# MIC-DKFZ/MultiTalent

Measured on AMD Instinct MI355X. Metric: CT patches/s (48x192x192) train fwd+bwd, higher is better.
Workload: dtype f32; 1 GPU; Task009_Spleen Generic_UNet nc=2 softmax Dice+CE; batch_per_gpu=2, global_batch=2, parallelism=dp1, step=fwd+loss+bwd+clip12+SGD-nesterov, precision=fp32

## Files before the change

### include/mtseg.h

```cpp
#ifndef MTSEG_H
#define MTSEG_H

#include <stddef.h>
#include <stdint.h>

#ifdef __cplusplus
extern "C" {
#endif

#define MT_OK 0
#define MT_EINVAL (-1)
#define MT_EWORKSPACE (-2)
#define MT_EHIP (-3)
#define MT_EUNSUPPORTED (-4)

#define MT_ABI_VERSION 4
#define MT_MAX_CHUNKS 64

#define MT_F32 0
#define MT_BF16 1
#define MT_F16 2

typedef void* mt_stream_t;

// ... 90 lines not shown
                         long s_ci, long s_co, long s_kd, long s_kh, long s_kw, int accumulate,
                         void* workspace, size_t workspace_bytes, mt_stream_t stream);

typedef struct {
  mt_src_t src;
  int32_t N, Db, Hb, Wb;
  int32_t Di, Hi, Wi;
  int32_t siD, siH, siW;
  int32_t soD, soH, soW;
  int32_t Cin, Cout;
  const float* wpack;
  const float* bias;
  float* out; int32_t ocs;
  int32_t accumulate;
  float* stats_part;
  int32_t odtype;
  int32_t scatter;
  int32_t mma;
} mt_pointwise_t;
int mt_pointwise_fwd(const mt_pointwise_t* p, mt_stream_t stream);
int mt_pointwise_stats_blocks(const mt_pointwise_t* p);
int mt_pointwise_io_supported(const mt_pointwise_t* p);
int mt_pointwise_pack_layout(const mt_pointwise_t* p);
int mt_pointwise_kernel_name(const mt_pointwise_t* p, char* buf, size_t n);
int mt_pointwise_launch_shape(const mt_pointwise_t* p, int32_t shape[4]);
int mt_head_bwd_supported(int Cin, int Cout);
size_t mt_head_bwd_workspace(int N, long V, int Cin, int Cout);
int mt_head_bwd(const mt_src_t* x, const float* dy, int dycs, int N, long V, int Cin, int Cout, const float* wpack_bwd,
                float* dx, int dxcs, int dxdtype , int accumulate_dx, float* dw,
                long s_ci, long s_co, float* dbias, int accumulate_dw, int* dbias_done, void* ws, size_t ws_bytes, mt_stream_t stream);
int mt_head_bwd_io_supported(int xdtype, int xcs, int dxdtype, int dxcs, int Cin, int Cout);
int mt_head_bwd_kernel_name(const mt_src_t* x, int dycs, int N, long V, int Cin, int Cout, int dxcs, int dxdtype, char* buf, size_t n,
                            int* dbias_done);


int mt_inorm_finalize(const float* part, int N, int nsb, int C, double count, const float* gamma,
                      const float* beta, float eps, float* mean, float* rstd, float* scale, float* shift,
                      mt_stream_t stream);
int mt_inorm_lrelu_apply(const float* y, int ycs, const float* scale, const float* shift, float slope,
                         const float* res, int rcs, const float* rscale, const float* rshift, float rslope,
                         float* out, int ocs, int N, long V, int C, int dtype , mt_stream_t stream);
size_t mt_inorm_bwd_workspace(int N, long V, int C);
int mt_inorm_lrelu_bwd(float* g, int gcs, const float* y, int ycs, const float* mean, const float* rstd,
                       const float* gamma, const float* beta, float slope, int N, long V, int C,
                       float* dgamma, float* dbeta, float* dbias, const float* part, int part_nblk, int part_cs, int part_c0,
                       void* ws, size_t ws_bytes, int gdtype, int ydtype , mt_stream_t stream);
int mt_lrelu_bwd(float* g, int gcs, const float* y, int ycs, const float* scale, const float* shift,
                 float slope, const float* y2, int y2cs, const float* scale2, const float* shift2,
                 float slope2, float* gcopy, int gcopycs, int N, long V, int C, int gdtype , int ydtype ,
                 mt_stream_t stream);
int mt_lrelu_bwd_stats_blocks(long V, int C);
int mt_lrelu_bwd_stats(float* g, const float* y, const float* scale, const float* shift, float slope,
                       const float* y2, const float* scale2, const float* shift2, float slope2, float* gcopy,
                       const float* mean, const float* rstd, float* part, int N, long V, int C, int gdtype ,
                       int ydtype , mt_stream_t stream);
int mt_inorm_lrelu_apply_kernel_name(const float* y, int ycs, const float* res, int rcs, const float* out, int ocs, int N, long V, int C,
                                     int dtype, char* buf, size_t n);
int mt_inorm_lrelu_bwd_kernel_name(const float* g, int gcs, const float* y, int ycs, const float* mean, const float* rstd, int N, long V, int C,
                                   const float* part, int part_nblk, int part_cs, int part_c0, int gdtype, int ydtype,
                                   char* buf, size_t n, int* own_reduce, int* block);
int mt_lrelu_bwd_kernel_name(const float* g, int gcs, const float* y, int ycs, const float* y2, int y2cs, const float* gcopy, int gcopycs,
                             int N, long V, int C, int gdtype, int ydtype, char* buf, size_t n);
int mt_lrelu_bwd_stats_kernel_name(const float* g, const float* y, const float* y2, const float* gcopy, const float* mean, const float* rstd,
                                   const float* part, int N, long V, int C, int gdtype, int ydtype, char* buf, size_t n);
size_t mt_channel_sum_workspace(int N, long V, int C);
int mt_channel_sum(const float* x, int xcs, int N, long V, int C, float* out, int accumulate,
// ... 194 lines not shown
```

### multitalent_amd/_lib.py

```python
import ctypes as C
import os

_HERE = os.path.dirname(os.path.abspath(__file__))
LIB_PATH = os.path.join(_HERE, os.environ.get('MT_LIB_VARIANT', 'libmtseg_hip.so'))

MT_MAX_CHUNKS = 64
c_float_p = C.POINTER(C.c_float)


class mt_src_t(C.Structure):
    _fields_ = [('ptr', C.c_void_p), ('cs', C.c_int32), ('C', C.c_int32), ('scale', C.c_void_p),
                ('shift', C.c_void_p), ('slope', C.c_float), ('dtype', C.c_int32)]


class mt_bwd_stats_t(C.Structure):
    _fields_ = [('y', C.c_void_p), ('mean', C.c_void_p), ('rstd', C.c_void_p), ('gamma', C.c_void_p), ('beta', C.c_void_p),
                ('ycs', C.c_int32), ('c0', C.c_int32), ('C', C.c_int32), ('slope', C.c_float)]


class mt_conv3d_t(C.Structure):
    _fields_ = [('src', mt_src_t * 2), ('nsrc', C.c_int32),
                ('N', C.c_int32), ('Di', C.c_int32), ('Hi', C.c_int32), ('Wi', C.c_int32),
                ('dilD', C.c_int32), ('dilH', C.c_int32), ('dilW', C.c_int32),
                ('Do', C.c_int32), ('Ho', C.c_int32), ('Wo', C.c_int32),
# ... 44 lines not shown

_vp, _i, _l, _f, _d, _sz = C.c_void_p, C.c_int, C.c_long, C.c_float, C.c_double, C.c_size_t
_P = C.POINTER

SIGNATURES = {
    'mt_last_error': (C.c_char_p, []),
    'mt_abi_version': (_i, []),
    'mt_probe_device': (_i, [_vp, _sz, _P(_i), C.c_char_p, _sz, _vp]),
    'mt_pack_conv_weights': (_i, [_vp, _vp, _P(_sz), _i, _i, _i, _i, _i, _i, _l, _l, _l, _l, _l, _i, _i, _i, _vp, _vp]),
    'mt_conv3d_fwd': (_i, [_P(mt_conv3d_t), _vp]),
    'mt_conv3d_stats_blocks': (_i, [_P(mt_conv3d_t)]),
    'mt_conv3d_ck': (_i, [_P(mt_conv3d_t)]),
    'mt_pack_desc_size': (_sz, []),
    'mt_pack_desc_fill': (_i, [_vp, _vp, _vp, _i, _i, _i, _i, _i, _i, _l, _l, _l, _l, _l, _i, _i, _i, _vp]),
    'mt_pack_batched': (_i, [_vp, _i, _vp]),
    'mt_conv3d_bwd_data_strided': (_i, [_P(mt_conv3d_t), _vp]),
    'mt_conv3d_bwd_data_strided_supported': (_i, [_P(mt_conv3d_t)]),
    'mt_downsample_seg_nearest': (_i, [_vp, _i, _i, _i, _i, _vp, _i, _i, _i, _i, _vp]),
    'mt_gaussian_blur_axis': (_i, [_vp, _vp, _i, _i, _i, _i, _i, _vp, _vp]),
    'mt_conv3d_pack_layout': (_i, [_P(mt_conv3d_t)]),
    'mt_conv3d_bwd_data_strided_pack_layout': (_i, [_P(mt_conv3d_t)]),
    'mt_conv3d_kernel_name': (_i, [_P(mt_conv3d_t), C.c_char_p, _sz]),
    'mt_conv3d_bwd_stats_supported': (_i, [_P(mt_conv3d_t)]),
    'mt_conv3d_bwd_weight_kernel_name': (_i, [_P(mt_conv3d_t), _P(mt_src_t), C.c_char_p, _sz]),
    'mt_conv3d_bwd_data_strided_kernel_name': (_i, [_P(mt_conv3d_t), C.c_char_p, _sz]),
    'mt_conv3d_bwd_weight_workspace': (_sz, [_P(mt_conv3d_t)]),
    'mt_conv3d_bwd_weight': (_i, [_P(mt_conv3d_t), _P(mt_src_t), _vp, _l, _l, _l, _l, _l, _i, _vp, _sz, _vp]),
    'mt_pointwise_fwd': (_i, [_P(mt_pointwise_t), _vp]),
    'mt_pointwise_stats_blocks': (_i, [_P(mt_pointwise_t)]),
    'mt_head_bwd_supported': (_i, [_i, _i]),
    'mt_head_bwd_workspace': (_sz, [_i, _l, _i, _i]),
    'mt_head_bwd': (_i, [_P(mt_src_t), _vp, _i, _i, _l, _i, _i, _vp, _vp, _i, _i, _i, _vp, _l, _l, _vp, _i, _P(C.c_int), _vp, _sz, _vp]),
    'mt_head_bwd_io_supported': (_i, [_i, _i, _i, _i, _i, _i]),
    'mt_pointwise_io_supported': (_i, [_P(mt_pointwise_t)]),
    'mt_pointwise_pack_layout': (_i, [_P(mt_pointwise_t)]),
    'mt_pointwise_kernel_name': (_i, [_P(mt_pointwise_t), C.c_char_p, _sz]),
    'mt_pointwise_launch_shape': (_i, [_P(mt_pointwise_t), _P(C.c_int32)]),
    'mt_head_bwd_kernel_name': (_i, [_P(mt_src_t), _i, _i, _l, _i, _i, _i, _i, C.c_char_p, _sz, _P(C.c_int)]),
    'mt_inorm_finalize': (_i, [_vp, _i, _i, _i, _d, _vp, _vp, _f, _vp, _vp, _vp, _vp, _vp]),
    'mt_inorm_lrelu_apply': (_i, [_vp, _i, _vp, _vp, _f, _vp, _i, _vp, _vp, _f, _vp, _i, _i, _l, _i, _i, _vp]),
    'mt_inorm_bwd_workspace': (_sz, [_i, _l, _i]),
    'mt_inorm_lrelu_bwd': (_i, [_vp, _i, _vp, _i, _vp, _vp, _vp, _vp, _f, _i, _l, _i, _vp, _vp, _vp, _vp, _i, _i, _i, _vp, _sz, _i, _i, _vp]),
    'mt_lrelu_bwd': (_i, [_vp, _i, _vp, _i, _vp, _vp, _f, _vp, _i, _vp, _vp, _f, _vp, _i, _i, _l, _i, _i, _i, _vp]),
    'mt_lrelu_bwd_stats_blocks': (_i, [_l, _i]),
    'mt_lrelu_bwd_stats': (_i, [_vp, _vp, _vp, _vp, _f, _vp, _vp, _vp, _f, _vp, _vp, _vp, _vp, _i, _l, _i, _i, _i, _vp]),
    'mt_inorm_lrelu_apply_kernel_name': (_i, [_vp, _i, _vp, _i, _vp, _i, _i, _l, _i, _i, C.c_char_p, _sz]),
    'mt_inorm_lrelu_bwd_kernel_name': (_i, [_vp, _i, _vp, _i, _vp, _vp, _i, _l, _i, _vp, _i, _i, _i, _i, _i, C.c_char_p, _sz, _P(C.c_int), _P(C.c_int)]),
    'mt_lrelu_bwd_kernel_name': (_i, [_vp, _i, _vp, _i, _vp, _i, _vp, _i, _i, _l, _i, _i, _i, C.c_char_p, _sz]),
    'mt_lrelu_bwd_stats_kernel_name': (_i, [_vp, _vp, _vp, _vp, _vp, _vp, _vp, _i, _l, _i, _i, _i, C.c_char_p, _sz]),
    'mt_channel_sum_workspace': (_sz, [_i, _l, _i]),
    'mt_channel_sum': (_i, [_vp, _i, _i, _l, _i, _vp, _i, _vp, _sz, _i, _vp]),
    'mt_cast': (_i, [_vp, _i, _i, _vp, _i, _i, _l, _i, _i, _vp]),
    'mt_conv3d_io_supported': (_i, [_P(mt_conv3d_t)]),
    'mt_conv3d_bwd_data_strided_io_supported': (_i, [_P(mt_conv3d_t)]),
    'mt_conv3d_bwd_weight_io_supported': (_i, [_P(mt_conv3d_t), _P(mt_src_t)]),
    'mt_multitalent_loss_fwd': (_i, [_vp, _i, _vp, _i, _l, _i, _vp, _vp, _vp, _vp, _sz, _vp]),
    'mt_loss_workspace': (_sz, [_i, _l, _i]),
    'mt_multitalent_loss_bwd': (_i, [_vp, _i, _vp, _i, _l, _i, _vp, _vp, _vp, _vp, _i, _vp]),
    'mt_multitalent_hard_stats': (_i, [_vp, _i, _vp, _i, _l, _i, _vp, _vp, _vp, _vp, _sz, _vp]),
    'mt_hard_stats_workspace': (_sz, [_i, _i]),
    'mt_softmax_dice_ce_fwd': (_i, [_vp, _i, _vp, _i, _l, _i, _vp, _vp, _sz, _vp]),
    'mt_softmax_dice_ce_bwd': (_i, [_vp, _i, _vp, _i, _l, _i, _vp, _vp, _i, _vp]),
    'mt_loss_combine': (_i, [_vp, _vp, _i, _i, _i, _i, _vp, _vp, _i, _i, _f, _f, _f, _f, _f, _vp, _vp, _vp]),
    'mt_multitalent_loss_fwd_kernel_name': (_i, [_i, _l, _i, C.c_char_p, _sz, _P(C.c_long), _P(C.c_int)]),
    'mt_multitalent_loss_bwd_kernel_name': (_i, [_vp, _i, _vp, _i, _l, _i, C.c_char_p, _sz, _P(C.c_long), _P(C.c_int)]),
    'mt_softmax_dice_ce_kernel_name': (_i, [_i, _i, C.c_char_p, _sz]),
# ... 126 lines not shown
```

### multitalent_amd/csrc/head_bwd.hip

```cpp
#include "pw_common.h"
#include <stdio.h>

struct HeadBwdParams {
  mt_src_t x; const float* dy; int dycs; int N; long V; int Cin, Cout;
  const float* wpack; float* dx; int dxcs; int accumulate_dx;
  float* part; int nwaves; long ntiles;
};
template <int NCI, int XS = MT_F32, int OS = MT_F32, bool ST = false>
__global__ __launch_bounds__(256) void head_bwd_kernel(const HeadBwdParams P) {
  constexpr int XE = mt_ebytes<XS>(), OE = mt_ebytes<OS>();
  constexpr int HB_WF = 2048 + 1024 * NCI;
  __shared__ __attribute__((aligned(16))) float hb_img[ST ? 4 * HB_WF : 4];
  static_assert(!ST || 4 * HB_WF * sizeof(float) <= 65536, "head_bwd_kernel: the four wave images must fit the 64 KiB of static LDS (NCI <= 2)");
  const int tid = threadIdx.x, lane = tid & 63;
  const int wave = __builtin_amdgcn_readfirstlane(tid >> 6);
  float* const idy = hb_img + (ST ? wave * HB_WF : 0);
  float* const ixf = idy + (ST ? 2048 : 0);
  const int li = lane & 31, lhalf = lane >> 5;
  const int gw = blockIdx.x * 4 + wave;
  const mt_src_t& S = P.x;
  const bool aff = S.scale != nullptr;
  const float slope = aff ? S.slope : 1.f;
  const int nchunks = (P.Cout + 15) / 16;
  f32x4 wb[NCI][4][2];
// ... 236 lines not shown
  const int row = (j & 3) + 8 * (j >> 2) + 4 * (lane >> 5), col = lane & 31;
  const int ci = t * 32 + row, co = n * 32 + col;
  const bool is_bias = (R.Cin % 32) != 0 && t == R.nci - 1 && row == 31;
  if (co >= R.Cout || (ci >= R.Cin && !is_bias)) return;
  double a = 0.0;
  for (int sl = 0; sl < HB_SLICES; ++sl) a += R.tmp[(size_t)sl * per + e];
  const float s = (float)a;
  if (is_bias) { if (R.dbias != nullptr) R.dbias[co] = R.accumulate ? R.dbias[co] + s : s; return; }
  float* o = R.dw + (long)ci * R.s_ci + (long)co * R.s_co;
  *o = R.accumulate ? *o + s : s;
}

#define HN_BLOCKS 1024
template <int CIN, int ST>
__device__ __forceinline__ void hn_row_from_lds(const char* row, float (&x)[CIN + 2]) {
  if constexpr (ST == MT_F32) {
#pragma unroll
    for (int q = 0; q < CIN / 2; ++q) { const float2 t = *(const float2*)(row + q * 8); x[2 * q] = t.x; x[2 * q + 1] = t.y; }
  } else {
#pragma unroll
    for (int q = 0; q < CIN / 2; ++q) { const unsigned d = *(const unsigned*)(row + q * 4); x[2 * q] = mt_lo16<ST>(d); x[2 * q + 1] = mt_hi16<ST>(d); }
  }
}
template <int CIN, int ST>
__device__ __forceinline__ void hn_row_to_lds(char* row, const float (&x)[CIN + 2]) {
  if constexpr (ST == MT_F32) {
#pragma unroll
    for (int q = 0; q < CIN / 2; ++q) { float2 t; t.x = x[2 * q]; t.y = x[2 * q + 1]; *(float2*)(row + q * 8) = t; }
  } else {
#pragma unroll
    for (int q = 0; q < CIN / 2; ++q) *(unsigned*)(row + q * 4) = mt_pk16<ST>(x[2 * q], x[2 * q + 1]);
  }
}
template <int CIN, int NCO, int XS = MT_F32, int OS = MT_F32>
__global__ __launch_bounds__(256) void head_bwd_narrow_kernel(const HeadBwdParams P) {
  static_assert(CIN % 2 == 0, "channel pairs");
  __shared__ __attribute__((aligned(16))) float hn_img[4 * 64 * CIN];
  constexpr int XE = mt_ebytes<XS>(), OE = mt_ebytes<OS>();
  constexpr int NP = NCO * CIN + NCO;
  __shared__ __attribute__((aligned(16))) float sw[NCO][CIN + 2], ssc[CIN + 2], ssh[CIN + 2];
  __shared__ float red[4][NP];
  const int tid = threadIdx.x, lane = tid & 63;
  const int wave = __builtin_amdgcn_readfirstlane(tid >> 6);
  const mt_src_t& S = P.x;
  const bool aff = S.scale != nullptr;
  const float slope = aff ? S.slope : 1.f;
  for (int i = tid; i < NCO * CIN; i += 256) {
    const int co = i / CIN, ci = i - co * CIN;
    sw[co][ci] = co < P.Cout ? P.wpack[ci * 4 + co] : 0.f;
  }
  float part[NP];
#pragma unroll
  for (int k = 0; k < NP; ++k) part[k] = 0.f;
  const long per_sample_blocks = HN_BLOCKS / P.N > 0 ? HN_BLOCKS / P.N : 1;
  const int nb = (int)(blockIdx.x / per_sample_blocks);
  if (nb < P.N) {
    const long b = blockIdx.x - (long)nb * per_sample_blocks;
    for (int i = tid; i < CIN; i += 256) {
      ssc[i] = aff ? S.scale[(size_t)nb * S.C + i] : 1.f;
      ssh[i] = aff ? S.shift[(size_t)nb * S.C + i] : 0.f;
    }
    __syncthreads();
    const size_t xs = (size_t)P.V * CIN;
    __amdgpu_buffer_rsrc_t ra = __builtin_amdgcn_make_buffer_rsrc((void*)((const char*)S.ptr + (size_t)nb * xs * XE), 0, (int)(xs * XE), 0x00020000);
    __amdgpu_buffer_rsrc_t rx = __builtin_amdgcn_make_buffer_rsrc((void*)((char*)P.dx + (size_t)nb * xs * OE), 0, (int)(xs * OE), 0x00020000);
    const float* dyp = P.dy + (size_t)nb * P.V * P.dycs;
    constexpr int ROWX = CIN * XE, ROWO = CIN * OE;
    constexpr int NPX = 64 * ROWX / 16, NPO = 64 * ROWO / 16;
    char* const img = (char*)hn_img + wave * (64 * CIN * 4);
    for (long v0 = b * 256 + wave * 64; v0 < P.V; v0 += per_sample_blocks * 256) {
      const long v = v0 + lane;
      const bool vok = v < P.V;
      float x[CIN + 2], old[CIN + 2], dy[NCO];
      {
        uint4 pc[(NPX + 63) / 64];
#pragma unroll
        for (int k = 0; k < (NPX + 63) / 64; ++k) {
          const int p = k * 64 + lane;
          pc[k] = __builtin_bit_cast(uint4, __builtin_amdgcn_raw_buffer_load_b128(ra, p < NPX ? (int)(v0 * ROWX) + p * 16 : (int)0x80000000, 0, 0));
        }
#pragma unroll
        for (int k = 0; k < (NPX + 63) / 64; ++k) {
          const int p = k * 64 + lane;
          if (p < NPX) *(uint4*)(img + p * 16) = pc[k];
        }
        __builtin_amdgcn_s_waitcnt(0xc07f);
        __builtin_amdgcn_wave_barrier();
        hn_row_from_lds<CIN, XS>(img + lane * ROWX, x);
        __builtin_amdgcn_s_waitcnt(0xc07f);
        __builtin_amdgcn_wave_barrier();
      }
      if (P.accumulate_dx) {
        uint4 pc[(NPO + 63) / 64];
#pragma unroll
        for (int k = 0; k < (NPO + 63) / 64; ++k) {
          const int p = k * 64 + lane;
          pc[k] = __builtin_bit_cast(uint4, __builtin_amdgcn_raw_buffer_load_b128(rx, p < NPO ? (int)(v0 * ROWO) + p * 16 : (int)0x80000000, 0, 0));
        }
#pragma unroll
        for (int k = 0; k < (NPO + 63) / 64; ++k) {
          const int p = k * 64 + lane;
          if (p < NPO) *(uint4*)(img + p * 16) = pc[k];
        }
        __builtin_amdgcn_s_waitcnt(0xc07f);
        __builtin_amdgcn_wave_barrier();
        hn_row_from_lds<CIN, OS>(img + lane * ROWO, old);
        __builtin_amdgcn_s_waitcnt(0xc07f);
        __builtin_amdgcn_wave_barrier();
      }
#pragma unroll
      for (int co = 0; co < NCO; ++co) dy[co] = (vok && co < P.Cout) ? dyp[v * P.dycs + co] : 0.f;
      float dx[CIN + 2];
#pragma unroll
      for (int ci = 0; ci < CIN; ++ci) {
        const float t = fmaf(x[ci], ssc[ci], ssh[ci]);
        const float a = fmaxf(t, t * slope);
        float g = P.accumulate_dx ? old[ci] : 0.f;
#pragma unroll
        for (int co = 0; co < NCO; ++co) {
          g = fmaf(dy[co], sw[co][ci], g);
          part[co * CIN + ci] = fmaf(a, dy[co], part[co * CIN + ci]);
        }
        dx[ci] = g;
      }
#pragma unroll
      for (int co = 0; co < NCO; ++co) part[NCO * CIN + co] += dy[co];
      hn_row_to_lds<CIN, OS>(img + lane * ROWO, dx);
      __builtin_amdgcn_s_waitcnt(0xc07f);
      __builtin_amdgcn_wave_barrier();
#pragma unroll
      for (int k = 0; k < (NPO + 63) / 64; ++k) {
        const int p = k * 64 + lane;
        if (p < NPO) {
          const uint4 q = *(const uint4*)(img + p * 16);
          __builtin_amdgcn_raw_buffer_store_b128(__builtin_bit_cast(__attribute__((ext_vector_type(4))) unsigned, q), rx, (int)(v0 * ROWO) + p * 16, 0, 0);
        }
      }
      __builtin_amdgcn_s_waitcnt(0xc07f);
      __builtin_amdgcn_wave_barrier();
    }
  }
#pragma unroll
  for (int k = 0; k < NP; ++k) {
    float s = part[k];
#pragma unroll
    for (int off = 32; off > 0; off >>= 1) s += __shfl_xor(s, off, 64);
    if (lane == 0) red[wave][k] = s;
  }
  __syncthreads();
  for (int k = tid; k < NP; k += 256) P.part[(size_t)blockIdx.x * NP + k] = (red[0][k] + red[1][k]) + (red[2][k] + red[3][k]);
}
__global__ __launch_bounds__(64) void head_narrow_reduce_kernel(const float* part, int nblocks, int np, int Cin, int Cout, int nco, float* dw, long s_ci,
                                                               long s_co, float* dbias, int accumulate) {
  const int k = blockIdx.x;
  double s = 0.0;
  for (int b = threadIdx.x; b < nblocks; b += 64) s += (double)part[(size_t)b * np + k];
  s = mt_wave_sum_d(s);
  if (threadIdx.x != 0) return;
  const int co = k < nco * Cin ? k / Cin : k - nco * Cin, ci = k < nco * Cin ? k - co * Cin : -1;
  if (co >= Cout) return;
  if (ci >= 0) { float* o = dw + (long)ci * s_ci + (long)co * s_co; *o = accumulate ? *o + (float)s : (float)s; }
  else if (dbias != nullptr) dbias[co] = accumulate ? dbias[co] + (float)s : (float)s;
}

extern "C" int mt_head_bwd_supported(int Cin, int Cout) { return Cin >= 1 && Cin <= 32 && Cout >= 1 && Cout <= 64; }
extern "C" int mt_head_bwd_io_supported(int xdtype, int xcs, int dxdtype, int dxcs, int Cin, int Cout) {
  if (xdtype == MT_F32 && dxdtype == MT_F32) return 1;
  if (!(mt_is16(xdtype) && dxdtype == MT_BF16)) return 0;
  return ((Cin & 1) || (xcs & 1) || (dxcs & 1)) ? 0 : 1;
}
static inline int head_bwd_waves(int N, long V) {
  const long ntiles = (long)N * ((V + 31) / 32);
  long w = ntiles / 32;
  if (w > 256 * 4 * 4) w = 256 * 4 * 4;
  if (w < 4) w = 4;
  return (int)((w + 3) / 4 * 4);
}
static inline size_t head_bwd_per(int Cin) { return (size_t)((Cin + 31) / 32) * 2 * 1024; }
static inline size_t head_bwd_tiled_bytes(int nwaves, size_t per) { return (size_t)nwaves * per * sizeof(float) + HB_SLICES * per * sizeof(double) + 64; }
static inline size_t head_bwd_narrow_bytes(int nblocks, int np) { return (size_t)nblocks * np * sizeof(float); }
struct HeadBwdChoice {
  bool narrow, staged;
  int tiles;
// ... 26 lines not shown
  return MT_OK;
}
extern "C" size_t mt_head_bwd_workspace(int N, long V, int Cin, int Cout) {
  if (!(Cin >= 1 && Cin <= 64 && Cout >= 1 && Cout <= 64)) return 0;
  const size_t tiled = head_bwd_tiled_bytes(head_bwd_waves(N, V), head_bwd_per(Cin));
  const size_t narrow = (Cout <= 4) ? head_bwd_narrow_bytes(HN_BLOCKS, 4 * 32 + 4) : 0;
  return tiled > narrow ? tiled : narrow;
}
extern "C" int mt_head_bwd_kernel_name(const mt_src_t* x, int dycs, int N, long V, int Cin, int Cout, int dxcs, int dxdtype, char* buf, size_t n,
                                       int* dbias_done) {
  MT_REQUIRE(buf != nullptr && n > 0, "head_bwd_kernel_name: no buffer");
  HeadBwdChoice c;
  if (int rc = head_bwd_resolve(x, dycs, N, V, Cin, Cout, nullptr, dxcs, dxdtype, c)) return rc;
  if (c.narrow) snprintf(buf, n, "head_bwd_narrow_kernel<%d, %d, %d, %d>", c.tiles, c.nco, c.xs, c.os);
  else snprintf(buf, n, "head_bwd_kernel<%d, %d, %d, %s>", c.tiles, c.xs, c.os, c.staged ? "true" : "false");
  if (dbias_done != nullptr) *dbias_done = c.dbias_done;
  return MT_OK;
}

template <int CIN, int NCO>
static void head_bwd_launch_narrow(const HeadBwdChoice& c, const HeadBwdParams& P, hipStream_t st) {
  const dim3 g(c.nblocks);
  if (c.xs == MT_F16) hipLaunchKernelGGL((head_bwd_narrow_kernel<CIN, NCO, MT_F16, MT_BF16>), g, dim3(256), 0, st, P);
  else if (c.xs == MT_BF16) hipLaunchKernelGGL((head_bwd_narrow_kernel<CIN, NCO, MT_BF16, MT_BF16>), g, dim3(256), 0, st, P);
  else hipLaunchKernelGGL((head_bwd_narrow_kernel<CIN, NCO>), g, dim3(256), 0, st, P);
}
template <int NCI, bool ST>
static void head_bwd_launch_tiled(const HeadBwdChoice& c, const HeadBwdParams& P, hipStream_t st) {
  const dim3 g(c.nwaves / 4);
  if (c.xs == MT_F16) hipLaunchKernelGGL((head_bwd_kernel<NCI, MT_F16, MT_BF16, ST>), g, dim3(256), 0, st, P);
  else if (c.xs == MT_BF16) hipLaunchKernelGGL((head_bwd_kernel<NCI, MT_BF16, MT_BF16, ST>), g, dim3(256), 0, st, P);
  else hipLaunchKernelGGL((head_bwd_kernel<NCI, MT_F32, MT_F32, ST>), g, dim3(256), 0, st, P);
}
extern "C" int mt_head_bwd(const mt_src_t* x, const float* dy, int dycs, int N, long V, int Cin, int Cout, const float* wpack_bwd,
                           float* dx, int dxcs, int dxdtype, int accumulate_dx, float* dw, long s_ci, long s_co, float* dbias, int accumulate_dw,
                           int* dbias_done, void* ws, size_t ws_bytes, mt_stream_t stream) {
  MT_REQUIRE(dy && wpack_bwd && dx && dw, "head_bwd: null / empty argument");
  HeadBwdChoice c;
  if (int rc = head_bwd_resolve(x, dycs, N, V, Cin, Cout, dx, dxcs, dxdtype, c)) return rc;
  if (ws == nullptr || ws_bytes < mt_head_bwd_workspace(N, V, Cin, Cout)) { mt_set_error("head_bwd: workspace too small"); return MT_EWORKSPACE; }
  hipStream_t st = (hipStream_t)stream;
  HeadBwdParams P;
  P.x = *x; P.dy = dy; P.dycs = dycs; P.N = N; P.V = V; P.Cin = Cin; P.Cout = Cout; P.wpack = wpack_bwd;
  P.dx = dx; P.dxcs = dxcs; P.accumulate_dx = accumulate_dx; P.part = (float*)ws;
  if (c.narrow) {
    MT_REQUIRE(head_bwd_narrow_bytes(c.nblocks, c.np) <= ws_bytes, "head_bwd: workspace too small for the narrow form");
    if (c.tiles == 30 && c.nco == 2) head_bwd_launch_narrow<30, 2>(c, P, st);
    else if (c.tiles == 30) head_bwd_launch_narrow<30, 4>(c, P, st);
    else if (c.nco == 2) head_bwd_launch_narrow<32, 2>(c, P, st);
    else head_bwd_launch_narrow<32, 4>(c, P, st);
    hipLaunchKernelGGL(head_narrow_reduce_kernel, dim3(c.np), dim3(64), 0, st, (const float*)ws, c.nblocks, c.np, Cin, Cout, c.nco, dw, s_ci, s_co, dbias, accumulate_dw);
    MT_CHECK_LAUNCH("head_bwd_narrow");
  } else {
    P.nwaves = c.nwaves; P.ntiles = (long)N * ((V + 31) / 32);
    if (c.staged) { if (c.tiles == 1) head_bwd_launch_tiled<1, true>(c, P, st); else head_bwd_launch_tiled<2, true>(c, P, st); }
    else { if (c.tiles == 1) head_bwd_launch_tiled<1, false>(c, P, st); else head_bwd_launch_tiled<2, false>(c, P, st); }
    MT_CHECK_LAUNCH("head_bwd");
    HeadBwdReduce R;
    R.part = (const float*)ws; R.nwaves = c.nwaves; R.nci = c.tiles; R.Cin = Cin; R.Cout = Cout; R.dw = dw; R.s_ci = s_ci; R.s_co = s_co;
    R.dbias = dbias; R.accumulate = accumulate_dw;
    R.tmp = (double*)(((uintptr_t)((float*)ws + (size_t)c.nwaves * c.per) + 7) & ~(uintptr_t)7);
    hipLaunchKernelGGL(head_bwd_reduce_a_kernel, dim3(mt_cdiv((long)c.per, 256), HB_SLICES), dim3(256), 0, st, R);
    hipLaunchKernelGGL(head_bwd_reduce_b_kernel, dim3(mt_cdiv((long)c.per, 256)), dim3(256), 0, st, R);
    MT_CHECK_LAUNCH("head_bwd_reduce");
  }
  if (dbias_done != nullptr) *dbias_done = c.dbias_done;
  return MT_OK;
}
```

### multitalent_amd/engine.py

```python
import contextlib
import os

import torch
from torch import nn

from . import ops
from .ops import Act, ConvGeom

LRELU_DEFAULT = 1e-2


class Val:

    def __init__(self, name, C):
        self.name, self.C = name, C
        self.act = None
        self.grad = None
        self.grad_init = False
        self.spatial = None


class _Op:
    params = ()

# ... 432 lines not shown
                assert not self.res.grad_init, "gradient of %s was written before its residual add ran backward" % self.res.name
                self.res.grad_init = True
            elif self.res.grad_init:
                self.res.grad.add_(g)
            else:
                self.res.grad.copy_(g)
                self.res.grad_init = True


class HeadOp(ConvNormOp):

    def __init__(self, name, src, out, conv):
        super().__init__(name, [src], out, conv, None, lrelu=False, pointwise=True)

    def _out_dtype(self, eng):
        return torch.float32

    def backward(self, eng):
        s0 = self.srcs[0]
        Cout = self.conv.out_channels
        if s0.grad is None or self.wb is None or not ops.head_bwd_supported(s0.C, Cout) or self.stride != (1, 1, 1):
            return super().backward(eng)
        g = self.out.grad
        assert g is not None and self.out.grad_init, "gradient of %s was never produced" % self.name
        gact = Act(g)
        dbias = eng.grad_of(self.conv.bias) if self.conv.bias is not None else None
        w = self.conv.weight
        st = _strides(w)
        io = eng.io(self.name + '.hbwd', [s0.act], [Act(s0.grad)], lambda ins, outs: (ins[0], outs[0]),
                    lambda xo: ops.head_bwd_io_supported(xo[0], xo[1], Cout))
        a, dx = io.build()
        io.pre()
        ws = eng.workspace(ops.head_bwd_workspace(a.N, a.V, s0.C, Cout))
        done = ops.head_bwd(a, gact, self.wb, dx, bool(io.accumulate(s0.grad_init)), eng.grad_of(w), st[0], st[1], dbias, False, ws)
        io.post(s0.grad_init)
        if dbias is not None and not done:
            ws2 = eng.workspace(ops.channel_sum_workspace(gact.N, gact.V, gact.C))
            ops.channel_sum(gact, dbias, False, ws2)
        s0.grad_init = True


class _IO:

    def __init__(self, eng, key, ins, outs, build, flags, grad_ins):
        self.eng, self._build = eng, build
        cast_in, cast_out = flags
        self.native = not (cast_in or cast_out)
        self._cin = [(a, g) for a, g in zip(ins, grad_ins) if cast_in and a.dtype != torch.float32]
        self.ins = [eng.as_fp32(a, geometry_only=True) if (cast_in and a.dtype != torch.float32) else a for a in ins]
        self._cout = []
        self.outs = []
        for i, o in enumerate(outs):
            if cast_out and o.dtype != torch.float32:
                t = Act(eng.buffer('%s.out%d' % (key, i), tuple(o.buf.shape[:4]) + (o.C,)))
                self._cout.append((t, o))
                self.outs.append(t)
            else:
                self.outs.append(o)

    def build(self):
        return self._build(self.ins, self.outs)

    def pre(self):
        for a, is_grad in self._cin:
            self.eng.as_fp32(a, reuse=not is_grad)

    def accumulate(self, acc):
# ... 527 lines not shown
```

### multitalent_amd/ops.py

```python
import ctypes as C
import os

import numpy as np
import torch

from . import _lib
from ._lib import mt_conv3d_t, mt_pointwise_t, mt_src_t


def _stream():
    return C.c_void_p(torch.cuda.current_stream().cuda_stream)


def _ptr(t):
    return C.c_void_p(t.data_ptr()) if t is not None else C.c_void_p(0)


def _check_dev(*ts):
    for t in ts:
        if t is not None and not t.is_cuda:
            raise RuntimeError("multitalent_amd ops require HIP device tensors (no CPU fallback)")


_DT_CODES = {torch.float32: _lib.MT_F32, torch.bfloat16: _lib.MT_BF16, torch.float16: _lib.MT_F16}
# ... 344 lines not shown
    p.out = out.data_ptr()
    p.ocs = out.cs
    p.odtype = out.dt
    p.accumulate = 1 if accumulate else 0
    p.stats_part = stats_part.data_ptr() if stats_part is not None else None
    p.mma = int(mma)
    return p


def pointwise_pack_layout(p):
    return _lib.load().mt_pointwise_pack_layout(C.byref(p))


def pointwise_kernel_name(p):
    buf = C.create_string_buffer(128)
    _lib.check(_lib.load().mt_pointwise_kernel_name(C.byref(p), buf, 128), 'pointwise_kernel_name')
    return buf.value.decode()


def pointwise_launch_shape(p):
    shape = (C.c_int32 * 4)()
    _lib.check(_lib.load().mt_pointwise_launch_shape(C.byref(p), shape), 'pointwise_launch_shape')
    return tuple(shape)


def pointwise_fwd(p):
    _lib.check(_lib.load().mt_pointwise_fwd(C.byref(p), _stream()), 'pointwise_fwd')


def head_bwd_supported(Cin, Cout):
    return bool(_lib.load().mt_head_bwd_supported(int(Cin), int(Cout)))


def head_bwd(x, dy, wpack_bwd, dx, accumulate_dx, dw, s_ci, s_co, dbias, accumulate_dw, ws):
    lib = _lib.load()
    assert dy.dt == _lib.MT_F32, "mt_head_bwd reads the fp32 loss gradient"
    xs = x.src()
    done = C.c_int(0)
    _lib.check(lib.mt_head_bwd(C.byref(xs), C.c_void_p(dy.data_ptr()), dy.cs, x.N, x.V, x.C, dy.C, _ptr(wpack_bwd),
                               C.c_void_p(dx.data_ptr()), dx.cs, dx.dt, int(accumulate_dx), _ptr(dw), int(s_ci), int(s_co), _ptr(dbias),
                               int(accumulate_dw), C.byref(done), _ptr(ws), ws.numel() * ws.element_size(), _stream()), 'head_bwd')
    return bool(done.value)


def head_bwd_kernel_name(x, dy, dx):
    xs = x.src()
    buf, done = C.create_string_buffer(128), C.c_int(0)
    _lib.check(_lib.load().mt_head_bwd_kernel_name(C.byref(xs), dy.cs, x.N, x.V, x.C, dy.C, dx.cs, dx.dt, buf, 128, C.byref(done)),
               'head_bwd_kernel_name')
    return buf.value.decode(), bool(done.value)


def head_bwd_io_supported(x, dx, Cout):
    return bool(_lib.load().mt_head_bwd_io_supported(x.dt, x.cs, dx.dt, dx.cs, x.C, int(Cout)))


def head_bwd_workspace(N, V, Cin, Cout):
    return _lib.load().mt_head_bwd_workspace(int(N), int(V), int(Cin), int(Cout))


def pointwise_stats_blocks(p):
    return _lib.load().mt_pointwise_stats_blocks(C.byref(p))


def inorm_finalize(part, N, nsb, Cn, count, gamma, beta, eps, mean, rstd, scale, shift):
    _lib.check(_lib.load().mt_inorm_finalize(_ptr(part), N, nsb, Cn, float(count), _ptr(gamma), _ptr(beta), float(eps),
                                             _ptr(mean), _ptr(rstd), _ptr(scale), _ptr(shift), _stream()), 'inorm_finalize')


def inorm_lrelu_apply(y, out, res=None):
    _lib.check(_lib.load().mt_inorm_lrelu_apply(
        C.c_void_p(y.data_ptr()), y.cs, _ptr(y.scale), _ptr(y.shift), y.slope,
        C.c_void_p(res.data_ptr()) if res is not None else None, res.cs if res is not None else 0,
        _ptr(res.scale) if res is not None else None, _ptr(res.shift) if res is not None else None,
        res.slope if res is not None else 1.0,
# ... 1157 lines not shown
```

Baseline: 67.17 patches/s.

## Fuse InstanceNorm backward statistics into the segmentation head backward kernel

```diff
diff --git a/include/mtseg.h b/include/mtseg.h
--- a/include/mtseg.h
+++ b/include/mtseg.h
@@ -146,6 +146,11 @@
 int mt_head_bwd_io_supported(int xdtype, int xcs, int dxdtype, int dxcs, int Cin, int Cout);
 int mt_head_bwd_kernel_name(const mt_src_t* x, int dycs, int N, long V, int Cin, int Cout, int dxcs, int dxdtype, char* buf, size_t n,
                             int* dbias_done);
+int mt_head_bwd_stats_blocks(const mt_src_t* x, int dycs, int N, long V, int Cin, int Cout, int dxcs, int dxdtype);
+int mt_head_bwd_stats(const mt_src_t* x, const float* dy, int dycs, int N, long V, int Cin, int Cout, const float* wpack_bwd,
+                      float* dx, int dxcs, int dxdtype, int accumulate_dx, float* dw, long s_ci, long s_co, float* dbias,
+                      int accumulate_dw, int* dbias_done, void* ws, size_t ws_bytes, const float* mean, const float* rstd,
+                      float* part, mt_stream_t stream);
 
 
 int mt_inorm_finalize(const float* part, int N, int nsb, int C, double count, const float* gamma,
diff --git a/multitalent_amd/_lib.py b/multitalent_amd/_lib.py
--- a/multitalent_amd/_lib.py
+++ b/multitalent_amd/_lib.py
@@ -100,6 +100,9 @@
     'mt_head_bwd_workspace': (_sz, [_i, _l, _i, _i]),
     'mt_head_bwd': (_i, [_P(mt_src_t), _vp, _i, _i, _l, _i, _i, _vp, _vp, _i, _i, _i, _vp, _l, _l, _vp, _i, _P(C.c_int), _vp, _sz, _vp]),
     'mt_head_bwd_io_supported': (_i, [_i, _i, _i, _i, _i, _i]),
+    'mt_head_bwd_stats_blocks': (_i, [_P(mt_src_t), _i, _i, _l, _i, _i, _i, _i]),
+    'mt_head_bwd_stats': (_i, [_P(mt_src_t), _vp, _i, _i, _l, _i, _i, _vp, _vp, _i, _i, _i, _vp, _l, _l, _vp, _i, _P(C.c_int), _vp, _sz, _vp, _vp, _vp,
+                               _vp]),
     'mt_pointwise_io_supported': (_i, [_P(mt_pointwise_t)]),
     'mt_pointwise_pack_layout': (_i, [_P(mt_pointwise_t)]),
     'mt_pointwise_kernel_name': (_i, [_P(mt_pointwise_t), C.c_char_p, _sz]),
diff --git a/multitalent_amd/csrc/head_bwd.hip b/multitalent_amd/csrc/head_bwd.hip
--- a/multitalent_amd/csrc/head_bwd.hip
+++ b/multitalent_amd/csrc/head_bwd.hip
@@ -292,10 +292,12 @@
     for (int q = 0; q < CIN / 2; ++q) *(unsigned*)(row + q * 4) = mt_pk16<ST>(x[2 * q], x[2 * q + 1]);
   }
 }
-template <int CIN, int NCO, int XS = MT_F32, int OS = MT_F32>
-__global__ __launch_bounds__(256) void head_bwd_narrow_kernel(const HeadBwdParams P) {
+struct HeadBwdStats { const float* mean; const float* rstd; float* part; };
+template <int CIN, int NCO, int XS, int OS, bool BST>
+__device__ __forceinline__ void head_bwd_narrow_body(const HeadBwdParams& P, const HeadBwdStats& B) {
   static_assert(CIN % 2 == 0, "channel pairs");
-  __shared__ __attribute__((aligned(16))) float hn_img[4 * 64 * CIN];
+  static_assert(!BST || (XS == MT_F32 && OS == MT_F32 && 2 * CIN <= 64), "the statistics walk fp32 images, 2 CIN lanes");
+  __shared__ __attribute__((aligned(16))) float hn_img[(BST ? 8 : 4) * 64 * CIN];
   constexpr int XE = mt_ebytes<XS>(), OE = mt_ebytes<OS>();
   constexpr int NP = NCO * CIN + NCO;
   __shared__ __attribute__((aligned(16))) float sw[NCO][CIN + 2], ssc[CIN + 2], ssh[CIN + 2];
@@ -312,8 +314,11 @@
   float part[NP];
 #pragma unroll
   for (int k = 0; k < NP; ++k) part[k] = 0.f;
+  float b1 = 0.f, b2 = 0.f;
   const long per_sample_blocks = HN_BLOCKS / P.N > 0 ? HN_BLOCKS / P.N : 1;
   const int nb = (int)(blockIdx.x / per_sample_blocks);
+  char* const img = (char*)hn_img + wave * (64 * CIN * 4);
+  char* const imgx = BST ? (char*)hn_img + (4 + wave) * (64 * CIN * 4) : img;
   if (nb < P.N) {
     const long b = blockIdx.x - (long)nb * per_sample_blocks;
     for (int i = tid; i < CIN; i += 256) {
@@ -321,13 +326,17 @@
       ssh[i] = aff ? S.shift[(size_t)nb * S.C + i] : 0.f;
     }
     __syncthreads();
+    float bsc = 0.f, bsh = 0.f, bmu = 0.f, brs = 0.f;
+    if constexpr (BST) {
+      const int c = lane % CIN;
+      bsc = ssc[c]; bsh = ssh[c]; bmu = B.mean[(size_t)nb * CIN + c]; brs = B.rstd[(size_t)nb * CIN + c];
+    }
     const size_t xs = (size_t)P.V * CIN;
     __amdgpu_buffer_rsrc_t ra = __builtin_amdgcn_make_buffer_rsrc((void*)((const char*)S.ptr + (size_t)nb * xs * XE), 0, (int)(xs * XE), 0x00020000);
     __amdgpu_buffer_rsrc_t rx = __builtin_amdgcn_make_buffer_rsrc((void*)((char*)P.dx + (size_t)nb * xs * OE), 0, (int)(xs * OE), 0x00020000);
     const float* dyp = P.dy + (size_t)nb * P.V * P.dycs;
     constexpr int ROWX = CIN * XE, ROWO = CIN * OE;
     constexpr int NPX = 64 * ROWX / 16, NPO = 64 * ROWO / 16;
-    char* const img = (char*)hn_img + wave * (64 * CIN * 4);
     for (long v0 = b * 256 + wave * 64; v0 < P.V; v0 += per_sample_blocks * 256) {
       const long v = v0 + lane;
       const bool vok = v < P.V;
@@ -342,11 +351,11 @@
 #pragma unroll
         for (int k = 0; k < (NPX + 63) / 64; ++k) {
           const int p = k * 64 + lane;
-          if (p < NPX) *(uint4*)(img + p * 16) = pc[k];
+          if (p < NPX) *(uint4*)(imgx + p * 16) = pc[k];
         }
         __builtin_amdgcn_s_waitcnt(0xc07f);
         __builtin_amdgcn_wave_barrier();
-        hn_row_from_lds<CIN, XS>(img + lane * ROWX, x);
+        hn_row_from_lds<CIN, XS>(imgx + lane * ROWX, x);
         __builtin_amdgcn_s_waitcnt(0xc07f);
         __builtin_amdgcn_wave_barrier();
       }
@@ -396,6 +405,21 @@
           __builtin_amdgcn_raw_buffer_store_b128(__builtin_bit_cast(__attribute__((ext_vector_type(4))) unsigned, q), rx, (int)(v0 * ROWO) + p * 16, 0, 0);
         }
       }
+      if constexpr (BST) {
+        if (lane < 2 * CIN) {
+          const float* gi = (const float*)img;
+          const float* yi = (const float*)imgx;
+#pragma unroll 8
+          for (int j = 0; j < 32; ++j) {
+            const float gq = gi[j * 2 * CIN + lane], yq = yi[j * 2 * CIN + lane];
+            const float t = fmaf(yq, bsc, bsh);
+            const float zh = (yq - bmu) * brs;
+            const float dz = t > 0.f ? gq : gq * slope;
+            b1 += dz;
+            b2 = fmaf(dz, zh, b2);
+          }
+        }
+      }
       __builtin_amdgcn_s_waitcnt(0xc07f);
       __builtin_amdgcn_wave_barrier();
     }
@@ -407,8 +431,27 @@
     for (int off = 32; off > 0; off >>= 1) s += __shfl_xor(s, off, 64);
     if (lane == 0) red[wave][k] = s;
   }
+  if constexpr (BST) {
+    if (lane < 2 * CIN) { ((float*)img)[lane * 2] = b1; ((float*)img)[lane * 2 + 1] = b2; }
+  }
   __syncthreads();
   for (int k = tid; k < NP; k += 256) P.part[(size_t)blockIdx.x * NP + k] = (red[0][k] + red[1][k]) + (red[2][k] + red[3][k]);
+  if constexpr (BST) {
+    if (tid < 2 * CIN) {
+      float w[4];
+#pragma unroll
+      for (int q = 0; q < 4; ++q) w[q] = hn_img[q * (64 * CIN) + tid] + hn_img[q * (64 * CIN) + 2 * CIN + tid];
+      B.part[(size_t)blockIdx.x * (2 * CIN) + tid] = (w[0] + w[1]) + (w[2] + w[3]);
+    }
+  }
+}
+template <int CIN, int NCO, int XS = MT_F32, int OS = MT_F32>
+__global__ __launch_bounds__(256) void head_bwd_narrow_kernel(const HeadBwdParams P) {
+  head_bwd_narrow_body<CIN, NCO, XS, OS, false>(P, HeadBwdStats{nullptr, nullptr, nullptr});
+}
+template <int CIN, int NCO>
+__global__ __launch_bounds__(256) void head_bwd_narrow_stats_kernel(const HeadBwdParams P, const HeadBwdStats B) {
+  head_bwd_narrow_body<CIN, NCO, MT_F32, MT_F32, true>(P, B);
 }
 __global__ __launch_bounds__(64) void head_narrow_reduce_kernel(const float* part, int nblocks, int np, int Cin, int Cout, int nco, float* dw, long s_ci,
                                                                long s_co, float* dbias, int accumulate) {
@@ -501,20 +544,29 @@
   else if (c.xs == MT_BF16) hipLaunchKernelGGL((head_bwd_kernel<NCI, MT_BF16, MT_BF16, ST>), g, dim3(256), 0, st, P);
   else hipLaunchKernelGGL((head_bwd_kernel<NCI, MT_F32, MT_F32, ST>), g, dim3(256), 0, st, P);
 }
-extern "C" int mt_head_bwd(const mt_src_t* x, const float* dy, int dycs, int N, long V, int Cin, int Cout, const float* wpack_bwd,
-                           float* dx, int dxcs, int dxdtype, int accumulate_dx, float* dw, long s_ci, long s_co, float* dbias, int accumulate_dw,
-                           int* dbias_done, void* ws, size_t ws_bytes, mt_stream_t stream) {
+static inline bool head_bwd_serves_stats(const mt_src_t* x, const HeadBwdChoice& c) {
+  return c.narrow && c.tiles == 30 && c.xs == MT_F32 && c.os == MT_F32 && x->scale != nullptr && x->shift != nullptr;
+}
+static int head_bwd_run(const mt_src_t* x, const float* dy, int dycs, int N, long V, int Cin, int Cout, const float* wpack_bwd,
+                        float* dx, int dxcs, int dxdtype, int accumulate_dx, float* dw, long s_ci, long s_co, float* dbias, int accumulate_dw,
+                        int* dbias_done, void* ws, size_t ws_bytes, const HeadBwdStats* B, mt_stream_t stream) {
   MT_REQUIRE(dy && wpack_bwd && dx && dw, "head_bwd: null / empty argument");
   HeadBwdChoice c;
   if (int rc = head_bwd_resolve(x, dycs, N, V, Cin, Cout, dx, dxcs, dxdtype, c)) return rc;
   if (ws == nullptr || ws_bytes < mt_head_bwd_workspace(N, V, Cin, Cout)) { mt_set_error("head_bwd: workspace too small"); return MT_EWORKSPACE; }
+  MT_REQUIRE(B == nullptr || (head_bwd_serves_stats(x, c) && B->mean && B->rstd && B->part),
+             "head_bwd_stats: this head does not compute the statistics (ask mt_head_bwd_stats_blocks)");
   hipStream_t st = (hipStream_t)stream;
   HeadBwdParams P;
   P.x = *x; P.dy = dy; P.dycs = dycs; P.N = N; P.V = V; P.Cin = Cin; P.Cout = Cout; P.wpack = wpack_bwd;
   P.dx = dx; P.dxcs = dxcs; P.accumulate_dx = accumulate_dx; P.part = (float*)ws;
   if (c.narrow) {
     MT_REQUIRE(head_bwd_narrow_bytes(c.nblocks, c.np) <= ws_bytes, "head_bwd: workspace too small for the narrow form");
-    if (c.tiles == 30 && c.nco == 2) head_bwd_launch_narrow<30, 2>(c, P, st);
+    if (B != nullptr) {
+      if (c.nco == 2) hipLaunchKernelGGL((head_bwd_narrow_stats_kernel<30, 2>), dim3(c.nblocks), dim3(256), 0, st, P, *B);
+      else hipLaunchKernelGGL((head_bwd_narrow_stats_kernel<30, 4>), dim3(c.nblocks), dim3(256), 0, st, P, *B);
+    }
+    else if (c.tiles == 30 && c.nco == 2) head_bwd_launch_narrow<30, 2>(c, P, st);
     else if (c.tiles == 30) head_bwd_launch_narrow<30, 4>(c, P, st);
     else if (c.nco == 2) head_bwd_launch_narrow<32, 2>(c, P, st);
     else head_bwd_launch_narrow<32, 4>(c, P, st);
@@ -536,3 +588,23 @@
   if (dbias_done != nullptr) *dbias_done = c.dbias_done;
   return MT_OK;
 }
+extern "C" int mt_head_bwd(const mt_src_t* x, const float* dy, int dycs, int N, long V, int Cin, int Cout, const float* wpack_bwd,
+                           float* dx, int dxcs, int dxdtype, int accumulate_dx, float* dw, long s_ci, long s_co, float* dbias, int accumulate_dw,
+                           int* dbias_done, void* ws, size_t ws_bytes, mt_stream_t stream) {
+  return head_bwd_run(x, dy, dycs, N, V, Cin, Cout, wpack_bwd, dx, dxcs, dxdtype, accumulate_dx, dw, s_ci, s_co, dbias, accumulate_dw, dbias_done,
+                      ws, ws_bytes, nullptr, stream);
+}
+extern "C" int mt_head_bwd_stats_blocks(const mt_src_t* x, int dycs, int N, long V, int Cin, int Cout, int dxcs, int dxdtype) {
+  HeadBwdChoice c;
+  if (head_bwd_resolve(x, dycs, N, V, Cin, Cout, nullptr, dxcs, dxdtype, c) != MT_OK) return 0;
+  return head_bwd_serves_stats(x, c) ? c.nblocks / N : 0;
+}
+extern "C" int mt_head_bwd_stats(const mt_src_t* x, const float* dy, int dycs, int N, long V, int Cin, int Cout, const float* wpack_bwd,
+                                 float* dx, int dxcs, int dxdtype, int accumulate_dx, float* dw, long s_ci, long s_co, float* dbias,
+                                 int accumulate_dw, int* dbias_done, void* ws, size_t ws_bytes, const float* mean, const float* rstd,
+                                 float* part, mt_stream_t stream) {
+  MT_REQUIRE(mean && rstd && part, "head_bwd_stats: null argument");
+  const HeadBwdStats B{mean, rstd, part};
+  return head_bwd_run(x, dy, dycs, N, V, Cin, Cout, wpack_bwd, dx, dxcs, dxdtype, accumulate_dx, dw, s_ci, s_co, dbias, accumulate_dw, dbias_done,
+                      ws, ws_bytes, &B, stream);
+}
diff --git a/multitalent_amd/engine.py b/multitalent_amd/engine.py
--- a/multitalent_amd/engine.py
+++ b/multitalent_amd/engine.py
@@ -488,7 +488,17 @@
         a, dx = io.build()
         io.pre()
         ws = eng.workspace(ops.head_bwd_workspace(a.N, a.V, s0.C, Cout))
-        done = ops.head_bwd(a, gact, self.wb, dx, bool(io.accumulate(s0.grad_init)), eng.grad_of(w), st[0], st[1], dbias, False, ws)
+        prod = eng.producer.get(id(s0))
+        part = None
+        if (io.native and eng.pending.get(id(s0), 0) == 1 and isinstance(prod, ConvNormOp) and not isinstance(prod, HeadOp)
+                and prod.norm is not None and a.mean is not None):
+            nblk = ops.head_bwd_stats_blocks(a, gact, dx)
+            if nblk > 0:
+                part = eng.buffer(self.name + '.bwdpart', (a.N, nblk, a.C, 2))
+        done = ops.head_bwd(a, gact, self.wb, dx, bool(io.accumulate(s0.grad_init)), eng.grad_of(w), st[0], st[1], dbias, False, ws,
+                            stats_part=part)
+        if part is not None:
+            prod.bwd_part = (part, 0)
         io.post(s0.grad_init)
         if dbias is not None and not done:
             ws2 = eng.workspace(ops.channel_sum_workspace(gact.N, gact.V, gact.C))
diff --git a/multitalent_amd/ops.py b/multitalent_amd/ops.py
--- a/multitalent_amd/ops.py
+++ b/multitalent_amd/ops.py
@@ -400,15 +400,27 @@
     return bool(_lib.load().mt_head_bwd_supported(int(Cin), int(Cout)))
 
 
-def head_bwd(x, dy, wpack_bwd, dx, accumulate_dx, dw, s_ci, s_co, dbias, accumulate_dw, ws):
+def head_bwd(x, dy, wpack_bwd, dx, accumulate_dx, dw, s_ci, s_co, dbias, accumulate_dw, ws, stats_part=None):
     lib = _lib.load()
     assert dy.dt == _lib.MT_F32, "mt_head_bwd reads the fp32 loss gradient"
     xs = x.src()
     done = C.c_int(0)
-    _lib.check(lib.mt_head_bwd(C.byref(xs), C.c_void_p(dy.data_ptr()), dy.cs, x.N, x.V, x.C, dy.C, _ptr(wpack_bwd),
-                               C.c_void_p(dx.data_ptr()), dx.cs, dx.dt, int(accumulate_dx), _ptr(dw), int(s_ci), int(s_co), _ptr(dbias),
-                               int(accumulate_dw), C.byref(done), _ptr(ws), ws.numel() * ws.element_size(), _stream()), 'head_bwd')
+    args = (C.byref(xs), C.c_void_p(dy.data_ptr()), dy.cs, x.N, x.V, x.C, dy.C, _ptr(wpack_bwd),
+            C.c_void_p(dx.data_ptr()), dx.cs, dx.dt, int(accumulate_dx), _ptr(dw), int(s_ci), int(s_co), _ptr(dbias),
+            int(accumulate_dw), C.byref(done), _ptr(ws), ws.numel() * ws.element_size())
+    if stats_part is not None:
+        assert x.mean is not None and x.rstd is not None, "head_bwd(stats_part=...): x carries no InstanceNorm statistics"
+        assert tuple(stats_part.shape) == (x.N, head_bwd_stats_blocks(x, dy, dx), x.C, 2) and stats_part.is_contiguous() \
+            and stats_part.dtype == torch.float32
+        _lib.check(lib.mt_head_bwd_stats(*args, _ptr(x.mean), _ptr(x.rstd), _ptr(stats_part), _stream()), 'head_bwd_stats')
+    else:
+        _lib.check(lib.mt_head_bwd(*args, _stream()), 'head_bwd')
     return bool(done.value)
+
+
+def head_bwd_stats_blocks(x, dy, dx):
+    xs = x.src()
+    return int(_lib.load().mt_head_bwd_stats_blocks(C.byref(xs), dy.cs, x.N, x.V, x.C, dy.C, dx.cs, dx.dt))
 
 
 def head_bwd_kernel_name(x, dy, dx):
```

Measured after the change: 67.48 patches/s (median of 6 runs). Within noise of the previous version (+0.5%).
